# dfm/george

Measured on AMD Instinct MI355X. Metric: gp_compute_plus_log_likelihood_effective_tflops, higher is better.
Workload: dtype f64; 1 GPU; N=65536 1-D sorted uniform(0,10) x, var(y)*ExpSquaredKernel(1.0), yerr=0.1, dense Cholesky fp64 (BasicSolver path): compute()+log_likelihood(); N=65536, kernel=ExpSquared, solver=dense-cholesky, parallelism=1gpu

## Files before the change

### george_amd/_native.py

```python
import ctypes as C
import os

import numpy as np

_HERE = os.path.dirname(os.path.abspath(__file__))
LIB_PATH = os.path.join(_HERE, "csrc", "libgeorge_amd.so")

GH_MAX_AXES, GH_MAX_NDIM, GH_MAX_PARAMS, GH_MAX_METRIC = 8, 16, 4, 36
GH_MAX_NODES, GH_MAX_GRAD, GH_MAX_STACK = 64, 64, 8
GH_OK, GH_ERR_NOT_PD, GH_ERR_BAD_ARG, GH_ERR_HIP, GH_ERR_NOT_COMPUTED, GH_ERR_DIM, GH_ERR_NOMEM, GH_ERR_RANK = range(8)
GH_OP_LEAF, GH_OP_SUM, GH_OP_PRODUCT = 0, 1, 2


class gh_knode(C.Structure):
    _fields_ = [
        ("op", C.c_int32), ("kernel_type", C.c_int32), ("metric_type", C.c_int32),
        ("ndim", C.c_int32), ("naxes", C.c_int32), ("blocked", C.c_int32),
        ("n_params", C.c_int32), ("n_metric", C.c_int32),
        ("axes", C.c_int32 * GH_MAX_AXES),
        ("params", C.c_double * GH_MAX_PARAMS),
        ("constant", C.c_double),
        ("metric", C.c_double * GH_MAX_METRIC),
        ("min_block", C.c_double * GH_MAX_AXES),
        ("max_block", C.c_double * GH_MAX_AXES),
    ]


class gh_chol_opts(C.Structure):
    _fields_ = [("device", C.c_int32), ("nb", C.c_int32), ("profile", C.c_int32),
                ("lookahead", C.c_int32), ("reserved", C.c_int32 * 4)]


class gh_chol_profile(C.Structure):
    _fields_ = [("ms_total", C.c_double), ("ms_build", C.c_double), ("ms_panel", C.c_double),
                ("ms_trailing", C.c_double), ("trailing_flops", C.c_double), ("n_trailing", C.c_int64),
                ("ms_solve", C.c_double), ("ms_update_union", C.c_double), ("update_flops", C.c_double),
                ("reserved", C.c_double * 2)]


class gh_hodlr_opts(C.Structure):
    _fields_ = [("device", C.c_int32), ("min_size", C.c_int32), ("seed", C.c_int32),
                ("max_rank", C.c_int32), ("tol", C.c_double), ("reserved", C.c_int32 * 4)]


class gh_mgpu_opts(C.Structure):
    _fields_ = [("n_dev", C.c_int32), ("devices", C.c_int32 * 16), ("pr", C.c_int32), ("pc", C.c_int32),
                ("nb", C.c_int32), ("transport", C.c_int32), ("flags", C.c_int32), ("reserved", C.c_int32 * 3)]


class gh_hodlr_mgpu_opts(C.Structure):
    _fields_ = [("n_dev", C.c_int32), ("devices", C.c_int32 * 16), ("min_size", C.c_int32), ("seed", C.c_int32),
                ("max_rank", C.c_int32), ("tol", C.c_double), ("reserved", C.c_int32 * 4)]


GH_MGPU_RCCL, GH_MGPU_COPY = 0, 1
GH_MGPU_PLAIN_CYCLIC, GH_MGPU_CHAIN_ONLY, GH_MGPU_TRACE, GH_MGPU_ONE_COMM = 1, 2, 4, 8

if not os.path.exists(LIB_PATH):
    raise ImportError(
        "george_amd: %s not found -- build the HIP extension first "
        "(python -c 'import __graft_entry__ as g; g.build()' or make -C george_amd/csrc)" % LIB_PATH)

def _share_hip_runtime_with_torch():
    if os.environ.get("GEORGE_AMD_HIP_RUNTIME", "") == "system":
        return
    try:
        import importlib.util
        spec = importlib.util.find_spec("torch")
        if spec is None or not spec.submodule_search_locations:
            return
        cand = os.path.join(list(spec.submodule_search_locations)[0], "lib", "libamdhip64.so")
        if os.path.exists(cand):
            C.CDLL(cand, mode=C.RTLD_GLOBAL)
    except Exception:
        pass


_share_hip_runtime_with_torch()
lib = C.CDLL(LIB_PATH)

_vp, _dp, _i64, _i32 = C.c_void_p, C.c_void_p, C.c_int64, C.c_int32

SIGNATURES = {
    "gh_device_count": (C.c_int, []),
    "gh_last_error": (C.c_char_p, []),
    "gh_version": (C.c_char_p, []),
    "gh_release_caches": (None, [C.c_int32]),
    "gh_set_cache_limit": (None, [C.c_int64]),
    "gh_microbench_mfma_f64": (C.c_int, [C.POINTER(C.c_double)]),
    "gh_microbench_hbm_copy": (C.c_int, [C.POINTER(C.c_double)]),
    "gh_debug_set_mfma": (C.c_int, [C.c_int]),
    "gh_debug_set_gemm_sp": (C.c_int, [C.c_int]),
    "gh_debug_set_adaptive_panels": (C.c_int, [C.c_int]),
    "gh_debug_set_build_on_chain": (C.c_int, [C.c_int]),
    "gh_debug_set_gemm_grouped": (C.c_int, [C.c_int]),
    "gh_debug_set_hodlr_passes": (C.c_int, [C.c_int]),
    "gh_debug_set_hodlr_leaf_gj": (C.c_int, [C.c_int]),
    "gh_debug_set_hodlr_wave_aca": (C.c_int, [C.c_int]),
    "gh_debug_set_hodlr_coop_wgs": (C.c_int, [C.c_int]),
    "gh_debug_set_hodlr_coop_lower": (C.c_int, [C.c_int]),
    "gh_debug_set_hodlr_lpt": (C.c_int, [C.c_int]),
    "gh_debug_set_hodlr_u_from_v": (C.c_int, [C.c_int]),
    "gh_debug_set_hodlr_core_fused": (C.c_int, [C.c_int]),
    "gh_debug_set_hodlr_coop_singles": (C.c_int, [C.c_int]),
    "gh_debug_set_hodlr_leaf_fused": (C.c_int, [C.c_int]),
    "gh_debug_set_hodlr_strip_cols": (C.c_int, [C.c_int]),
    "gh_debug_stream_overlap": (C.c_int, [_vp, C.POINTER(C.c_double), C.c_int]),
    "gh_debug_stream_dispatch": (C.c_int, [_vp, C.POINTER(C.c_double), C.c_int]),
    "gh_microbench_suite": (C.c_int, [C.POINTER(C.c_double), C.c_int]),
    "gh_microbench_mfma_f64_ceiling": (C.c_int, [C.POINTER(C.c_double), C.c_int]),
    "gh_kernel_create": (C.c_int, [C.POINTER(gh_knode), C.c_int, C.POINTER(_vp)]),
    "gh_kernel_destroy": (None, [_vp]),
    "gh_kernel_ndim": (C.c_int, [_vp]),
    "gh_kernel_size": (C.c_int, [_vp]),
    "gh_kernel_value_general": (C.c_int, [_vp, _dp, _i64, _dp, _i64, _dp]),
    "gh_kernel_value_symmetric": (C.c_int, [_vp, _dp, _i64, _dp]),
    "gh_kernel_value_diagonal": (C.c_int, [_vp, _dp, _dp, _i64, _dp]),
    "gh_kernel_gradient_general": (C.c_int, [_vp, _dp, _dp, _i64, _dp, _i64, _dp]),
    "gh_kernel_gradient_symmetric": (C.c_int, [_vp, _dp, _dp, _i64, _dp]),
    "gh_kernel_x1_gradient_general": (C.c_int, [_vp, _dp, _i64, _dp, _i64, _dp]),
    "gh_kernel_x2_gradient_general": (C.c_int, [_vp, _dp, _i64, _dp, _i64, _dp]),
    "gh_chol_create": (C.c_int, [C.POINTER(gh_chol_opts), C.POINTER(_vp)]),
    "gh_chol_destroy": (None, [_vp]),
    "gh_chol_compute": (C.c_int, [_vp, _vp, _dp, _i64, _i32, _dp, C.POINTER(C.c_double)]),
    "gh_chol_info": (_i64, [_vp]),
    "gh_chol_size": (_i64, [_vp]),
    "gh_chol_device_bytes": (_i64, [_vp]),
    "gh_chol_solve": (C.c_int, [_vp, _dp, _i64, _dp]),
    "gh_chol_dot_solve": (C.c_int, [_vp, _dp, C.POINTER(C.c_double)]),
    "gh_chol_apply_sqrt": (C.c_int, [_vp, _dp, _i64, _dp]),
    "gh_chol_get_inverse": (C.c_int, [_vp, _dp]),
    "gh_chol_predict": (C.c_int, [_vp, _vp, _dp, _dp, _i64, _dp, _dp, _dp]),
    "gh_chol_grad": (C.c_int, [_vp, _vp, _dp, _dp, _dp, _dp, _dp]),
    "gh_chol_objective": (C.c_int, [_vp, _vp, _dp, _i64, _i32, _dp, _dp, _dp, C.POINTER(C.c_double), C.POINTER(C.c_double),
                                    _dp, _dp, _dp]),
    "gh_chol_objective_batch": (C.c_int, [_vp, _vp, _dp, _i32, _dp, _i64, _i32, _dp, _dp, _dp, _dp, _dp]),
    "gh_chol_predict_batch": (C.c_int, [_vp, _vp, _dp, _i32, _dp, _i64, _i32, _dp, _dp, _dp, _i64, _dp, _dp, _dp, _dp, _dp,
                                        _dp]),
    "gh_chol_objective_grad_batch": (C.c_int, [_vp, _vp, _dp, _i32, _dp, _i64, _i32, _dp, _dp, _dp, _dp, _dp, _dp, _dp,
                                               _dp, _dp]),
    "gh_chol_factor_size": (_i64, [_vp]),
    "gh_chol_dinv_size": (_i64, [_vp]),
    "gh_chol_export_factor": (C.c_int, [_vp, _dp, _dp]),
    "gh_chol_import_factor": (C.c_int, [_vp, _i64, _i32, _dp, _dp, _dp, C.c_double]),
    "gh_chol_trim": (None, [_vp]),
    "gh_chol_release_buffers": (None, [_vp]),
    "gh_chol_get_profile": (C.c_int, [_vp, C.POINTER(gh_chol_profile)]),
    "gh_chol_get_update_intervals": (C.c_int, [_vp, _dp, _i32, C.POINTER(C.c_int32)]),
    "gh_hodlr_create": (C.c_int, [C.POINTER(gh_hodlr_opts), C.POINTER(_vp)]),
    "gh_hodlr_destroy": (None, [_vp]),
    "gh_hodlr_compute": (C.c_int, [_vp, _vp, _dp, _i64, _i32, _dp, C.POINTER(C.c_double)]),
    "gh_hodlr_solve": (C.c_int, [_vp, _dp, _i64, _dp]),
    "gh_hodlr_dot_solve": (C.c_int, [_vp, _dp, C.POINTER(C.c_double)]),
    "gh_hodlr_get_inverse": (C.c_int, [_vp, _dp]),
    "gh_hodlr_ranks": (C.c_int, [_vp, C.POINTER(C.c_int32), _i32, C.POINTER(C.c_int32)]),
    "gh_hodlr_predict": (C.c_int, [_vp, _vp, _dp, _dp, _i64, _dp, _dp, _dp]),
    "gh_hodlr_grad": (C.c_int, [_vp, _vp, _dp, _dp, _dp, _dp, _dp]),
    "gh_mgpu_create": (C.c_int, [C.POINTER(gh_mgpu_opts), C.POINTER(_vp)]),
    "gh_mgpu_destroy": (None, [_vp]),
    "gh_mgpu_compute": (C.c_int, [_vp, _vp, _dp, _i64, _i32, _dp, C.POINTER(C.c_double)]),
    "gh_mgpu_info": (_i64, [_vp]),
    "gh_mgpu_grid": (C.c_int, [_vp, C.POINTER(C.c_int32), C.POINTER(C.c_int32), C.POINTER(C.c_int32)]),
    "gh_mgpu_comm_mode": (C.c_int, [_vp]),
    "gh_mgpu_dot_solve": (C.c_int, [_vp, _dp, C.POINTER(C.c_double)]),
    "gh_mgpu_solve": (C.c_int, [_vp, _dp, _i64, _dp]),
    "gh_mgpu_owner": (C.c_int, [_vp, _i64, _i64]),
    "gh_mgpu_apply_sqrt": (C.c_int, [_vp, _dp, _i64, _dp]),
    "gh_mgpu_get_inverse": (C.c_int, [_vp, _dp]),
    "gh_mgpu_predict": (C.c_int, [_vp, _vp, _dp, _dp, _i64, _dp, _dp, _dp]),
    "gh_mgpu_get_trace": (C.c_int, [_vp, _dp, _i64, C.POINTER(C.c_int64)]),
    "gh_hodlr_mgpu_create": (C.c_int, [C.POINTER(gh_hodlr_mgpu_opts), C.POINTER(_vp)]),
    "gh_hodlr_mgpu_destroy": (None, [_vp]),
    "gh_hodlr_mgpu_compute": (C.c_int, [_vp, _vp, _dp, _i64, _i32, _dp, C.POINTER(C.c_double)]),
    "gh_hodlr_mgpu_solve": (C.c_int, [_vp, _dp, _i64, _dp]),
    "gh_hodlr_mgpu_dot_solve": (C.c_int, [_vp, _dp, C.POINTER(C.c_double)]),
    "gh_hodlr_mgpu_ranks": (C.c_int, [_vp, C.POINTER(C.c_int32), _i32, C.POINTER(C.c_int32)]),
# ... 63 lines not shown
```

### george_amd/csrc/gh_chol.hip

```cpp
#include <math.h>
#include <string.h>
#include <algorithm>
#include <chrono>
#include "gh_common.h"
#include "gh_device_util.h"
#include "gh_spin.h"
#include "../../include/george_amd_debug.h"

#define T 128
#define LP 129

__global__ __launch_bounds__(256) void potf2_inv_kernel(double* A, long lda, double* dinv,
                                                        long long* info, long long base) {
  __shared__ double s[T * LP];
  __shared__ int fail_at;
  const int tid = threadIdx.x;
  if (*info != 0) return;
  if (tid == 0) fail_at = -1;
  for (int idx = tid; idx < T * T; idx += 256) {
    const int i = idx >> 7, j = idx & 127;
    s[i * LP + j] = A[(long)i * lda + j];
  }
  __syncthreads();
  const int ty = tid >> 4, tx = tid & 15;
  for (int j = 0; j < T; ++j) {
    const double d = s[j * LP + j];
    if (!(d > 0.0)) {
      if (tid == 0) fail_at = j;
      break;
    }
    const double ajj = sqrt(d);
    __syncthreads();
    if (tid < T) {
      if (tid > j) s[tid * LP + j] /= ajj;
      else if (tid == j) s[j * LP + j] = ajj;
    }
    __syncthreads();
    for (int i = j + 1 + ((ty - (j + 1)) & 15); i < T; i += 16) {
      const double lij = s[i * LP + j];
      for (int k = j + 1 + ((tx - (j + 1)) & 15); k <= i; k += 16)
        s[i * LP + k] -= lij * s[k * LP + j];
    }
    __syncthreads();
  }
  __syncthreads();
  if (fail_at >= 0) {
    if (tid == 0) *info = base + fail_at + 1;
    return;
  }
  for (int idx = tid; idx < T * T; idx += 256) {
    const int i = idx >> 7, j = idx & 127;
    A[(long)i * lda + j] = (j <= i) ? s[i * LP + j] : 0.0;
  }
  __syncthreads();
  {
    volatile double* vs = s;
    const int c = tid >> 1, h = tid & 1;
    const double xc = 1.0 / vs[c * LP + c];
    for (int i = c + 1; i < T; ++i) {
      double acc = (h == 0) ? vs[i * LP + c] * xc : 0.0;
      for (int k = c + 1 + h; k < i; k += 2) acc += vs[i * LP + k] * vs[c * LP + k];
      acc += __shfl_xor(acc, 1, 64);
      const double xi = -acc / vs[i * LP + i];
      if (h == 0) vs[c * LP + i] = xi;
    }
  }
  __syncthreads();
  for (int idx = tid; idx < T * T; idx += 256) {
    const int i = idx >> 7, j = idx & 127;
    double v;
    if (j < i) v = s[j * LP + i];
    else if (j == i) v = 1.0 / s[i * LP + i];
    else v = 0.0;
    dinv[idx] = v;
  }
}


__global__ __launch_bounds__(256) void logdet_kernel(const double* A, long lda, long n, double* out, int accumulate) {
  __shared__ double sh[4];
  double v = 0.0;
  for (long i = threadIdx.x; i < n; i += 256) v += log(A[i * lda + i]);
  v = block_sum_256(v, sh);
  if (threadIdx.x == 0) out[0] = (accumulate ? out[0] : 0.0) + 2.0 * v;
}
__global__ __launch_bounds__(256) void dot_kernel(const double* a, const double* b, long n, double* out, const int* fail) {
  __shared__ double sh[4];
  double v = 0.0;
  for (long i = threadIdx.x; i < n; i += 256) v += a[i] * b[i];
// ... 264 lines not shown
  }
  red[wave][2 * lane] = acc.x;
  red[wave][2 * lane + 1] = acc.y;
  __syncthreads();
  if (tid < T) {
    double v = 0.0;
#pragma unroll
    for (int q = 0; q < 8; ++q) v += red[q][tid];
    wv[tid] = zv - v;
  }
  __syncthreads();
  acc = make_double2(0.0, 0.0);
#pragma unroll
  for (int q = 0; q < 16; ++q) { const double wr = wv[wave * 16 + q]; acc.x += dv[q].x * wr; acc.y += dv[q].y * wr; }
  __syncthreads();
  red[wave][2 * lane] = acc.x;
  red[wave][2 * lane + 1] = acc.y;
  __syncthreads();
  if (tid < T) {
    double v = 0.0;
#pragma unroll
    for (int q = 0; q < 8; ++q) v += red[q][tid];
    if (!chain_ready(v)) v = __longlong_as_double(0x7FF8000000000000LL);
    __hip_atomic_store(x + (long)b * T + tid, v, __ATOMIC_RELAXED, __HIP_MEMORY_SCOPE_AGENT);
  }
}

__global__ __launch_bounds__(256) void colreduce_kernel(const double* V, long ldv, long nrows, long rows_per,
                                                        const double* z, double* pmu, double* pvar, long ncols_p) {
  const long c = (long)blockIdx.x * 256 + threadIdx.x;
  if (c >= ncols_p) return;
  const long r0 = (long)blockIdx.y * rows_per;
  const long r1 = r0 + rows_per < nrows ? r0 + rows_per : nrows;
  double am = 0.0, av = 0.0;
  for (long r = r0; r < r1; ++r) {
    const double v = V[r * ldv + c];
    am += v * z[r];
    av += v * v;
  }
  pmu[(long)blockIdx.y * ncols_p + c] = am;
  pvar[(long)blockIdx.y * ncols_p + c] = av;
}
__global__ void colfinal_kernel(const double* pmu, const double* pvar, long nchunks, long ncols_p, long m,
                                double* mu, double* var ) {
  const long c = (long)blockIdx.x * blockDim.x + threadIdx.x;
  if (c >= m) return;
  double am = 0.0, av = 0.0;
  for (long s = 0; s < nchunks; ++s) { am += pmu[s * ncols_p + c]; av += pvar[s * ncols_p + c]; }
  mu[c] = am;
  if (var) var[c] -= av;
}
__global__ void fill_kernel(double* p, long n, double v) {
  for (long i = (long)blockIdx.x * blockDim.x + threadIdx.x; i < n; i += (long)gridDim.x * blockDim.x) p[i] = v;
}
__global__ void eye_kernel(double* p, long n, long ld) {
  const long i = (long)blockIdx.x * blockDim.x + threadIdx.x;
  if (i < n) p[i * ld + i] = 1.0;
}
__global__ void symmetrize_kernel(const double* in, long ldi, double* out, long ldo, long n) {
  const long idx = (long)blockIdx.x * blockDim.x + threadIdx.x;
  if (idx >= n * n) return;
  const long i = idx / n, j = idx % n;
  out[i * ldo + j] = (j <= i) ? in[i * ldi + j] : in[j * ldi + i];
}
__global__ void copy2d_kernel(const double* in, long ldi, double* out, long ldo, long rows, long cols) {
  const long idx = (long)blockIdx.x * blockDim.x + threadIdx.x;
  if (idx >= rows * cols) return;
  const long i = idx / cols, j = idx % cols;
  out[i * ldo + j] = in[i * ldi + j];
}

struct EvPair { hipEvent_t a, b; };

struct gh_chol {
  gh_chol_opts opts;
  hipStream_t st = nullptr;
  hipStream_t st2 = nullptr;
  hipStream_t st3 = nullptr;
  bool shared_streams = false;
  hipStream_t st4 = nullptr;
  hipEvent_t ev_diag[32] = {};
  hipEvent_t ev_aux = nullptr, ev_aux2 = nullptr;
  std::vector<hipEvent_t> ev_p, ev_w, ev_nf;
  hipStream_t st_mask = nullptr;
  hipStream_t tail = nullptr;


  int mask_reserved = -1;
  hipEvent_t ev_xfer = nullptr;
  hipEvent_t ev_sync[3] = {nullptr, nullptr, nullptr};
  int64_t n = 0, np = 0;
  int ndim = 0;
  bool computed = false;
  int64_t info = 0;
  double logdet = 0.0;
  GhBuf A, dinv, x, yerr, v0, v1, v2, scal, rhs, work, work2, scratch, chain;
  long long* d_info = nullptr;
  bool build_on_chain = false;
  GhBatchBufs* batch = nullptr;
  gh_chol_profile prof;
  std::vector<EvPair> ev_pool;
  size_t ev_used = 0;
  std::vector<size_t> ev_trailing, ev_panel, ev_update;
  std::vector<double> ev_update_flops;
  std::vector<double> upd_intervals;
  long next_ev() {
    if (ev_used == ev_pool.size()) {
      EvPair p;
      if (hipEventCreate(&p.a) != hipSuccess || hipEventCreate(&p.b) != hipSuccess) return -1;
      ev_pool.push_back(p);
    }
    return (long)ev_used++;
  }
  ~gh_chol() {
    for (auto& p : ev_pool) { (void)hipEventDestroy(p.a); (void)hipEventDestroy(p.b); }
    for (auto& e : ev_sync) if (e) (void)hipEventDestroy(e);
    if (ev_xfer) (void)hipEventDestroy(ev_xfer);
    if (ev_aux) (void)hipEventDestroy(ev_aux);
    if (ev_aux2) (void)hipEventDestroy(ev_aux2);
    for (auto* v : {&ev_p, &ev_w, &ev_nf}) for (auto e : *v) (void)hipEventDestroy(e);
    for (auto& e : ev_diag) if (e) (void)hipEventDestroy(e);
    if (st4 && !shared_streams) (void)hipStreamDestroy(st4);
    if (st3 && !shared_streams) (void)hipStreamDestroy(st3);
    if (st_mask && !shared_streams) (void)hipStreamDestroy(st_mask);


    if (st2 && !shared_streams) (void)hipStreamDestroy(st2);
    if (st && !shared_streams) (void)hipStreamDestroy(st);
    gh_batch_free(batch);
  }
};

#include <map>
#include <mutex>
namespace {
struct SharedStreams {
  hipStream_t q[4] = {nullptr, nullptr, nullptr, nullptr};
  bool made = false;
  bool main_crowded = false;
  std::map<int, hipStream_t> masked;
};
std::mutex g_ss_mu;
std::map<int, SharedStreams> g_ss;
}
namespace {
__global__ void place_spin_kernel(long long ticks) {
  const long long t0 = wall_clock64();
  while (wall_clock64() - t0 < ticks) {}
}
double dispatch_wait_ms(hipStream_t big, hipStream_t small) {
  (void)hipDeviceSynchronize();
  hipLaunchKernelGGL(place_spin_kernel, dim3(1 << 17), dim3(64), 0, big, 5000LL);
  const auto t0 = std::chrono::steady_clock::now();
  hipLaunchKernelGGL(place_spin_kernel, dim3(1), dim3(64), 0, small, 0LL);
  (void)hipStreamSynchronize(small);
  const double ms = std::chrono::duration<double, std::milli>(std::chrono::steady_clock::now() - t0).count();
  (void)hipDeviceSynchronize();
  return ms;
}
}
bool gh_streams_dispatch_independently(hipStream_t a, hipStream_t b) {
  if (!a || !b || a == b) return false;
  hipLaunchKernelGGL(place_spin_kernel, dim3(1), dim3(64), 0, a, 0LL);
  hipLaunchKernelGGL(place_spin_kernel, dim3(1), dim3(64), 0, b, 0LL);
  (void)hipDeviceSynchronize();
  const bool ok = dispatch_wait_ms(a, b) <= 0.3 && dispatch_wait_ms(b, a) <= 0.3;
  (void)hipGetLastError();
  return ok;
}
bool gh_shared_main_crowded(int device) {
  std::lock_guard<std::mutex> lk(g_ss_mu);
  auto it = g_ss.find(device);
  return it != g_ss.end() && it->second.main_crowded;
}
bool gh_shared_streams(int device, hipStream_t q[4]) {
  std::lock_guard<std::mutex> lk(g_ss_mu);
  SharedStreams& ss = g_ss[device];
  if (!ss.made) {
    ss.made = true;
    if (hipSetDevice(device) != hipSuccess) { (void)hipGetLastError(); return false; }
    gh_prime_device(device);
    if (hipStreamCreate(&ss.q[0]) != hipSuccess) { ss.q[0] = nullptr; (void)hipGetLastError(); }
    int lo = 0, hi = 0;
    (void)hipDeviceGetStreamPriorityRange(&lo, &hi);
    for (int i = 1; i < 4 && ss.q[0]; ++i)
      if (hipStreamCreateWithPriority(&ss.q[i], hipStreamNonBlocking, hi) != hipSuccess) { ss.q[i] = nullptr; (void)hipGetLastError(); break; }
    if (ss.q[0] && ss.q[1] && ss.q[2] && ss.q[3]) {
      for (int i = 0; i < 4; ++i) hipLaunchKernelGGL(place_spin_kernel, dim3(1), dim3(64), 0, ss.q[i], 0LL);
      (void)hipDeviceSynchronize();
      for (int i = 1; i < 4 && !ss.main_crowded; ++i)
        ss.main_crowded = dispatch_wait_ms(ss.q[0], ss.q[i]) > 0.3 || dispatch_wait_ms(ss.q[i], ss.q[0]) > 0.3;
      (void)hipGetLastError();
    }
  }
  for (int i = 0; i < 4; ++i) q[i] = ss.q[i];
  return ss.q[0] != nullptr;
}
hipStream_t gh_shared_masked_stream(int device, int reserve_cus) {
  std::lock_guard<std::mutex> lk(g_ss_mu);
  SharedStreams& ss = g_ss[device];
  auto it = ss.masked.find(reserve_cus);
  if (it != ss.masked.end()) return it->second;
  hipStream_t st = nullptr;
// ... 170 lines not shown
      GH_CHECK(gemm_nt(st, P, ld, P, ld, dj, T, rem, T, T, 1.0, 0.0, false));
      GH_CHECK(gemm_nt(st, blk(A, ld, j0 + T, j0 + T), ld, P, ld, P, ld, rem, rem, T, -1.0, 1.0, true));
    }
  }
  return GH_OK;
}
static int trsm_right(hipStream_t st, const double* L11, int64_t ld11, const double* dinv, double* A21, int64_t lda, int64_t m, int64_t n) {
  for (int64_t j0 = 0; j0 < n; j0 += T) {
    double* Xj = A21 + j0;
    if (j0 > 0)
      GH_CHECK(gemm_nt(st, Xj, lda, A21, lda, L11 + j0 * ld11, ld11, m, T, j0, -1.0, 1.0, false));
    GH_CHECK(gemm_nt(st, Xj, lda, Xj, lda, dinv + (j0 / T) * T * T, T, m, T, T, 1.0, 0.0, false));
  }
  return GH_OK;
}

static int launch_trsv_fwd_chain(const double* L, long ld, const double* dinv, int64_t nt, const double* w, double* z,
                                 unsigned* flags, hipStream_t st) {
  GH_HIP(hipMemsetAsync(flags + nt, 0, sizeof(unsigned), st));
  GH_HIP(hipMemsetAsync(z, 0xFF, (size_t)nt * T * sizeof(double), st));
  hipLaunchKernelGGL(trsv_fwd_chain_direct, dim3((unsigned)nt), dim3(CHAIN_THREADS), 0, st, L, ld, dinv, w, z, (int*)(flags + nt));
  GH_HIP(hipGetLastError());
  return GH_OK;
}
static int launch_trsv_bwd_chain(const double* L, long ld, const double* dinv, int64_t nt, const double* w, double* x,
                                 unsigned* flags, hipStream_t st) {
  GH_HIP(hipMemsetAsync(flags + nt, 0, sizeof(unsigned), st));
  GH_HIP(hipMemsetAsync(x, 0xFF, (size_t)nt * T * sizeof(double), st));
  hipLaunchKernelGGL(trsv_bwd_chain_direct, dim3((unsigned)nt), dim3(CHAIN_THREADS), 0, st, L, ld, dinv, (int)nt, w, x, (int*)(flags + nt));
  GH_HIP(hipGetLastError());
  return GH_OK;
}
extern "C" int gh_dev_potrf_block(double* a, int64_t lda, int64_t n, double* dinv, int64_t* info_dev, int64_t base_index, void* stream) {
  if (n % T) { gh_set_error("potrf_block: n must be a multiple of 128"); return GH_ERR_BAD_ARG; }
  struct Guard { bool prev; Guard() : prev(t_gemm_small_lds) { t_gemm_small_lds = true; } ~Guard() { t_gemm_small_lds = prev; } } guard;
  return potrf_block((hipStream_t)stream, a, lda, n, dinv, (long long*)info_dev, base_index);
}
extern "C" int gh_dev_trsm_right(const double* l11, int64_t ld11, const double* dinv, double* a21, int64_t lda, int64_t m, int64_t n, void* stream) {
  if (n % T || m % T) { gh_set_error("trsm_right: sizes must be multiples of 128"); return GH_ERR_BAD_ARG; }
  struct Guard { bool prev; Guard() : prev(t_gemm_small_lds) { t_gemm_small_lds = true; } ~Guard() { t_gemm_small_lds = prev; } } guard;
  return trsm_right((hipStream_t)stream, l11, ld11, dinv, a21, lda, m, n);
}
extern "C" int gh_dev_trsv_lower(const double* l, int64_t ldl, const double* dinv, int64_t n,
                                 const double* w, double* z, void* scratch, void* stream) {
  if (n % T || n <= 0 || !scratch) { gh_set_error("trsv_lower: n must be a positive multiple of 128"); return GH_ERR_BAD_ARG; }
  const int64_t nt = n / T;
  if (w == z) { gh_set_error("trsv_lower: w and z must not be the same array"); return GH_ERR_BAD_ARG; }
  return launch_trsv_fwd_chain(l, (long)ldl, dinv, nt, w, z, (unsigned*)scratch, (hipStream_t)stream);
}
extern "C" int gh_dev_trsv_lower_t(const double* l, int64_t ldl, const double* dinv, int64_t n,
                                   const double* w, double* x, void* scratch, void* stream) {
  if (n % T || n <= 0 || !scratch) { gh_set_error("trsv_lower_t: n must be a positive multiple of 128"); return GH_ERR_BAD_ARG; }
  const int64_t nt = n / T;
  if (w == x) { gh_set_error("trsv_lower_t: w and x must not be the same array"); return GH_ERR_BAD_ARG; }
  return launch_trsv_bwd_chain(l, (long)ldl, dinv, nt, w, x, (unsigned*)scratch, (hipStream_t)stream);
}
extern "C" int gh_dev_logdet_accum(const double* a, int64_t lda, int64_t n, double* out_dev, void* stream) {
  hipLaunchKernelGGL(logdet_kernel, dim3(1), dim3(256), 0, (hipStream_t)stream, a, (long)lda, (long)n, out_dev, 1);
  GH_HIP(hipGetLastError());
  return GH_OK;
}

static int64_t panel_width(const gh_chol* s) {
  if (s->opts.nb > 0) return s->opts.nb;
  return 1024;
}
#ifndef GH_WIDE_PANEL_MIN_TRAILING
#define GH_WIDE_PANEL_MIN_TRAILING 25600
#endif

static int g_build_on_chain = 1;
extern "C" int gh_debug_set_build_on_chain(int on) {
  const int prev = g_build_on_chain;
  g_build_on_chain = on ? 1 : 0;
  return prev;
}
static int g_adaptive_panels = 1;
extern "C" int gh_debug_set_adaptive_panels(int on) {
  const int prev = g_adaptive_panels;
  g_adaptive_panels = on < 0 ? 1 : on;
  return prev;
}
static std::vector<int64_t> panel_starts(const gh_chol* s) {
  std::vector<int64_t> pc;
  const int64_t np = s->np, nb = panel_width(s);
  const bool adaptive = s->opts.nb == 0 && g_adaptive_panels && !use_simple_potf2();
  for (int64_t k0 = 0; k0 < np;) {
    pc.push_back(k0);
    const int64_t bound = g_adaptive_panels > 1 ? g_adaptive_panels : GH_WIDE_PANEL_MIN_TRAILING;
    int64_t w = (adaptive && np - (k0 + 2 * nb) >= bound) ? 2 * nb : nb;
#ifdef GH_WIDE_PANEL_TIER2
    if (adaptive && np - (k0 + 4 * nb) >= GH_WIDE_PANEL_TIER2) w = 4 * nb;
#endif
    k0 += std::min<int64_t>(w, np - k0);
  }
  pc.push_back(np);
  return pc;
}

static int panel_step(gh_chol* s, hipStream_t st, int64_t k0, int64_t nb) {
  double* A = s->A.d();
  const int64_t np = s->np, ld = np;
  double* dinv = s->dinv.d() + (k0 / T) * T * T;
  const int64_t m = np - (k0 + nb);
  const bool on_panel_stream = (st == s->st2);
  if (!s->st3 || !on_panel_stream || m <= 0 || nb / T > 32 || use_simple_potf2()) {
    GH_CHECK(potrf_block(st, blk(A, ld, k0, k0), ld, nb, dinv, s->d_info, k0));
    if (m > 0) {
      GH_CHECK(trsm_right(st, blk(A, ld, k0, k0), ld, dinv, blk(A, ld, k0 + nb, k0), ld, m, nb));
    }
    return GH_OK;
  }
  hipStream_t sa = s->st3;
  double* Ak = blk(A, ld, k0, k0);
  double* B = blk(A, ld, k0 + nb, k0);
  for (int64_t j0 = 0; j0 < nb; j0 += T) {
    double* dj = dinv + (j0 / T) * T * T;
    GH_CHECK(gh_launch_potf2_mfma(blk(Ak, ld, j0, j0), ld, dj, s->d_info, k0 + j0, st));
    GH_HIP(hipEventRecord(s->ev_diag[j0 / T], st));
    GH_HIP(hipStreamWaitEvent(sa, s->ev_diag[j0 / T], 0));
    double* Xj = B + j0;
    if (j0 > 0) GH_CHECK(gemm_nt(sa, Xj, ld, B, ld, Ak + j0 * ld, ld, m, T, j0, -1.0, 1.0, false));
    GH_CHECK(gemm_nt(sa, Xj, ld, Xj, ld, dj, T, m, T, T, 1.0, 0.0, false));
    const int64_t rem = nb - (j0 + T);
    if (rem > 0) {
      double* P = blk(Ak, ld, j0 + T, j0);
      GH_CHECK(gemm_nt(st, P, ld, P, ld, dj, T, rem, T, T, 1.0, 0.0, false));
      GH_CHECK(gemm_nt(st, blk(Ak, ld, j0 + T, j0 + T), ld, P, ld, P, ld, rem, rem, T, -1.0, 1.0, true));
    }
  }
  GH_HIP(hipEventRecord(s->ev_aux, sa));
  GH_HIP(hipStreamWaitEvent(st, s->ev_aux, 0));
  return GH_OK;
}

static hipStream_t trailing_stream(gh_chol* s) {
  int want = s->np < 24576 ? 32 : 0;
  if (const char* e = getenv("GEORGE_AMD_RESERVE_CUS")) want = atoi(e);
  if (want <= 0 || want >= 128) return s->st;
  if (s->mask_reserved != want) {
    if (s->st_mask) { (void)hipStreamSynchronize(s->st_mask); if (!s->shared_streams) (void)hipStreamDestroy(s->st_mask); s->st_mask = nullptr; }
    s->mask_reserved = want;
    hipDeviceProp_t prop;
    if (hipGetDeviceProperties(&prop, s->opts.device) == hipSuccess && prop.multiProcessorCount > 2 * want) {
      const int ncu = prop.multiProcessorCount, words = (ncu + 31) / 32;
      std::vector<uint32_t> mask(words, 0u);
      for (int c = want; c < ncu; ++c) mask[c / 32] |= (1u << (c % 32));
      if (s->shared_streams) s->st_mask = gh_shared_masked_stream(s->opts.device, want);
      else if (hipExtStreamCreateWithCUMask(&s->st_mask, words, mask.data()) != hipSuccess) { s->st_mask = nullptr; (void)hipGetLastError(); }
    }
    if (s->st_mask && !s->ev_xfer && hipEventCreateWithFlags(&s->ev_xfer, hipEventDisableTiming) != hipSuccess) {
      (void)hipGetLastError(); if (!s->shared_streams) (void)hipStreamDestroy(s->st_mask); s->st_mask = nullptr;
    }
  }
  return s->st_mask ? s->st_mask : s->st;
}

static int factor_lookahead_deep(gh_chol* s, int depth) {
  hipStream_t sm = trailing_stream(s), sn = (depth == 1 && s->st3) ? s->st3 : s->st4;
  hipStream_t sp = s->st2;
#ifndef GH_FULLCHIP_MS
#define GH_FULLCHIP_MS 2.5
#endif
  const std::vector<int64_t> pc = panel_starts(s);
  auto wide_stream = [&](int j) -> hipStream_t {
    if (sm == s->st) return sm;
    const int cwj = j + depth + 1;
    if (j < 0 || cwj > (int)pc.size() - 2) return sm;
    const double m2 = (double)(s->np - pc[cwj]);
    const double ms = (m2 / T) * (m2 / T + 1.0) / 2.0 * 2.0 * T * T * (double)(pc[j + 1] - pc[j]) / 60e12 * 1e3;
    return ms > GH_FULLCHIP_MS ? s->st : sm;
  };
  hipStream_t sw_prev = nullptr;
  double* A = s->A.d();
  const int64_t np = s->np, ld = np;
  const int P = (int)pc.size() - 1;
  const bool prof = s->opts.profile != 0;
  while ((int)s->ev_p.size() < P) {
    hipEvent_t e[3];
    for (auto& x : e) GH_HIP(hipEventCreateWithFlags(&x, hipEventDisableTiming));
// ... 3 lines not shown
  auto nbc = [&](int c) { return pc[c + 1] - pc[c]; };
  auto narrow = [&](hipStream_t st, int j, int c) -> int {
    const double* Pj = blk(A, ld, c0(c), c0(j));
    const long eu = prof ? s->next_ev() : -1;
    if (eu >= 0) { GH_HIP(hipEventRecord(s->ev_pool[eu].a, st)); s->ev_update.push_back((size_t)eu); }
    GH_CHECK(gemm_nt(st, blk(A, ld, c0(c), c0(c)), ld, Pj, ld, Pj, ld, np - c0(c), nbc(c), nbc(j), -1.0, 1.0, false));
    if (eu >= 0) GH_HIP(hipEventRecord(s->ev_pool[eu].b, st));
    const double tr = (double)(np - c0(c)) / T, tc = (double)nbc(c) / T;
    const double fl = (tr * tc - tc * (tc - 1.0) / 2.0) * 2.0 * T * T * (double)nbc(j);
    s->prof.update_flops += fl;
    if (eu >= 0) s->ev_update_flops.push_back(fl);
    return GH_OK;
  };
  if (!s->build_on_chain) {
    GH_HIP(hipEventRecord(s->ev_sync[0], s->st));
    GH_HIP(hipStreamWaitEvent(sp, s->ev_sync[0], 0));
    GH_HIP(hipStreamWaitEvent(sn, s->ev_sync[0], 0));
    if (sm != s->st) GH_HIP(hipStreamWaitEvent(sm, s->ev_sync[0], 0));
  }
  for (int j = 0; j < P; ++j) {
    {
      const long ep = prof ? s->next_ev() : -1;
      if (ep >= 0) { GH_HIP(hipEventRecord(s->ev_pool[ep].a, sp)); s->ev_panel.push_back((size_t)ep); }
      t_gemm_small_lds = wide_stream(j >= 1 ? j - 1 : 0) == s->st;
      GH_CHECK(panel_step(s, sp, c0(j), nbc(j)));
      if (ep >= 0) GH_HIP(hipEventRecord(s->ev_pool[ep].b, sp));
      GH_HIP(hipEventRecord(s->ev_p[j], sp));
    }
    if (j + 1 >= P) break;
    const hipEvent_t prev = (j >= 1) ? (depth >= 2 ? s->ev_nf[j - 1] : s->ev_w[j - 1]) : nullptr;
    if (prev) GH_HIP(hipStreamWaitEvent(sp, prev, 0));
    GH_CHECK(narrow(sp, j, j + 1));
    const int last_near = std::min(j + depth, P - 1);
    if (j + 2 <= last_near || (depth >= 2 && j + 2 <= P - 1)) GH_HIP(hipStreamWaitEvent(sn, s->ev_p[j], 0));
    for (int c = j + 2; c <= last_near; ++c) {
      if (c == j + depth && j >= 1) GH_HIP(hipStreamWaitEvent(sn, s->ev_w[j - 1], 0));
      GH_CHECK(narrow(sn, j, c));
      if (c == j + 2) GH_HIP(hipEventRecord(s->ev_nf[j], sn));
    }
    if (depth >= 2 && j + 2 > last_near) GH_HIP(hipEventRecord(s->ev_nf[j], sn));
    const int cw = j + depth + 1;
    hipStream_t sw = wide_stream(j);
    if (sw_prev && sw_prev != sw && j >= 1) GH_HIP(hipStreamWaitEvent(sw, s->ev_w[j - 1], 0));
    sw_prev = sw;
    GH_HIP(hipStreamWaitEvent(sw, s->ev_p[j], 0));
    if (cw <= P - 1) {
      const int64_t kw = c0(cw), m2 = np - kw;
      const long et = prof ? s->next_ev() : -1;
      if (et >= 0) {
        GH_HIP(hipEventRecord(s->ev_pool[et].a, sw)); s->ev_trailing.push_back((size_t)et); s->ev_update.push_back((size_t)et);
        s->ev_update_flops.push_back((double)(m2 / T) * (m2 / T + 1) / 2.0 * 2.0 * T * T * (double)nbc(j));
      }
      const double* P2 = blk(A, ld, kw, c0(j));
      GH_CHECK(gemm_nt(sw, blk(A, ld, kw, kw), ld, P2, ld, P2, ld, m2, m2, nbc(j), -1.0, 1.0, true));
      if (et >= 0) GH_HIP(hipEventRecord(s->ev_pool[et].b, sw));
      const double tiles = (double)(m2 / T) * (m2 / T + 1) / 2.0;
      s->prof.trailing_flops += tiles * 2.0 * T * T * (double)nbc(j);
      s->prof.update_flops += tiles * 2.0 * T * T * (double)nbc(j);
      s->prof.n_trailing += 1;
    }
    GH_HIP(hipEventRecord(s->ev_w[j], sw));
  }
  const bool join_on_chain = !s->shared_streams || gh_shared_main_crowded(s->opts.device);
  if (sm != s->st && join_on_chain) {
    GH_HIP(hipEventRecord(s->ev_sync[2], sn));
    GH_HIP(hipStreamWaitEvent(sp, s->ev_sync[2], 0));
    GH_HIP(hipEventRecord(s->ev_xfer, sm));
    GH_HIP(hipStreamWaitEvent(sp, s->ev_xfer, 0));
    if (P >= 2) GH_HIP(hipStreamWaitEvent(sp, s->ev_w[P - 2], 0));
    s->tail = sp;
    return GH_OK;
  }
  GH_HIP(hipEventRecord(s->ev_sync[1], sp));
  GH_HIP(hipStreamWaitEvent(s->st, s->ev_sync[1], 0));
  GH_HIP(hipEventRecord(s->ev_sync[2], sn));
  GH_HIP(hipStreamWaitEvent(s->st, s->ev_sync[2], 0));
  if (sm != s->st) {
    GH_HIP(hipEventRecord(s->ev_xfer, sm));
    GH_HIP(hipStreamWaitEvent(s->st, s->ev_xfer, 0));
  }
  return GH_OK;
}

#ifndef GH_LOOKAHEAD_DEPTH
#define GH_LOOKAHEAD_DEPTH 1
#endif
static int lookahead_depth(const gh_chol* s) {
  return GH_LOOKAHEAD_DEPTH;
}

static int factor(gh_chol* s) {
  struct Guard { bool prev; Guard(bool v) : prev(t_gemm_small_lds) { t_gemm_small_lds = v; } ~Guard() { t_gemm_small_lds = prev; } }
      guard(s->opts.lookahead && s->st2 && trailing_stream(s) == s->st);
  if (s->opts.lookahead && s->st2 && s->st3 && s->st4 && s->np > panel_width(s)) return factor_lookahead_deep(s, lookahead_depth(s));
  hipStream_t st = s->st;
  double* A = s->A.d();
  const int64_t np = s->np, ld = np;
  const bool prof = s->opts.profile != 0;
  const std::vector<int64_t> pc = panel_starts(s);
  for (size_t pj = 0; pj + 1 < pc.size(); ++pj) {
    const int64_t k0 = pc[pj], nb = pc[pj + 1] - pc[pj];
    const long ep = prof ? s->next_ev() : -1;
    if (ep >= 0) { GH_HIP(hipEventRecord(s->ev_pool[ep].a, st)); s->ev_panel.push_back((size_t)ep); }
    GH_CHECK(potrf_block(st, blk(A, ld, k0, k0), ld, nb, s->dinv.d() + (k0 / T) * T * T, s->d_info, k0));
    const int64_t m = np - (k0 + nb);
    if (m > 0)
      GH_CHECK(trsm_right(st, blk(A, ld, k0, k0), ld, s->dinv.d() + (k0 / T) * T * T, blk(A, ld, k0 + nb, k0), ld, m, nb));
    if (ep >= 0) GH_HIP(hipEventRecord(s->ev_pool[ep].b, st));
    if (m > 0) {
      const long et = prof ? s->next_ev() : -1;
      if (et >= 0) { GH_HIP(hipEventRecord(s->ev_pool[et].a, st)); s->ev_trailing.push_back((size_t)et); }
      const double* P = blk(A, ld, k0 + nb, k0);
      GH_CHECK(gemm_nt(st, blk(A, ld, k0 + nb, k0 + nb), ld, P, ld, P, ld, m, m, nb, -1.0, 1.0, true));
      if (et >= 0) GH_HIP(hipEventRecord(s->ev_pool[et].b, st));
      const double tiles = (double)(m / T) * (m / T + 1) / 2.0;
      s->prof.trailing_flops += tiles * 2.0 * T * T * (double)nb;
      s->prof.n_trailing += 1;
    }
  }
  return GH_OK;
}

__global__ void prep_inputs_kernel(const double* xs, long nx, const double* es, long ne, double* xd, double* ed, long long* info) {
  const long i = (long)blockIdx.x * blockDim.x + threadIdx.x, stride = (long)gridDim.x * blockDim.x;
  for (long e = i; e < nx; e += stride) xd[e] = xs[e];
  for (long e = i; e < ne; e += stride) ed[e] = es[e];
  if (i == 0) *info = 0;
}

struct ComputeCtx { long e_all = -1, e_build = -1; };
static int compute_enqueue(gh_chol* s, gh_kernel* k, const double* x, int64_t n, int32_t ndim, const double* yerr, ComputeCtx& c) {
  if (!s || !k || !x || !yerr || n <= 0) { gh_set_error("bad argument to compute"); return GH_ERR_BAD_ARG; }
  if (ndim != k->ndim) { gh_set_error("dimension mismatch"); return GH_ERR_DIM; }
  GH_CHECK(set_device(s));
  GH_CHECK(k->upload());
  s->computed = false;
  s->info = 0;
  const int64_t np = gh_round_up(n, T);
  s->n = n; s->np = np; s->ndim = ndim;
  GH_CHECK(s->A.ensure((size_t)np * np * sizeof(double)));
  GH_CHECK(s->dinv.ensure((size_t)(np / T) * T * T * sizeof(double)));
  GH_CHECK(s->x.ensure((size_t)n * ndim * sizeof(double)));
  GH_CHECK(s->yerr.ensure((size_t)n * sizeof(double)));
  GH_CHECK(s->scal.ensure(256 * sizeof(double)));
  s->build_on_chain = g_build_on_chain && s->opts.lookahead && s->st2 && s->st3 && s->st4 && np > panel_width(s);
  hipStream_t st = s->build_on_chain ? s->st2 : s->st;
  memset(&s->prof, 0, sizeof(s->prof));
  s->ev_used = 0; s->ev_trailing.clear(); s->ev_panel.clear(); s->ev_update.clear(); s->ev_update_flops.clear();
  const bool prof = s->opts.profile != 0;
  c.e_all = prof ? s->next_ev() : -1;
  c.e_build = prof ? s->next_ev() : -1;
  if (c.e_all >= 0) GH_HIP(hipEventRecord(s->ev_pool[c.e_all].a, st));
  s->d_info = (long long*)(s->scal.d() + 2);
  if (gh_is_device_ptr(x) && gh_is_device_ptr(yerr)) {
    const long tot = (long)n * ndim;
    hipLaunchKernelGGL(prep_inputs_kernel, dim3((unsigned)std::min<long>((tot + 255) / 256, 1024)), dim3(256), 0, st,
                       x, tot, yerr, (long)n, s->x.d(), s->yerr.d(), s->d_info);
    GH_HIP(hipGetLastError());
  } else {
    GH_CHECK(gh_to_device(s->x.d(), x, (size_t)n * ndim, st));
    GH_CHECK(gh_to_device(s->yerr.d(), yerr, (size_t)n, st));
    GH_HIP(hipMemsetAsync(s->d_info, 0, sizeof(long long), st));
  }
  if (c.e_build >= 0) GH_HIP(hipEventRecord(s->ev_pool[c.e_build].a, st));
  GH_CHECK(gh_launch_kmat(k, s->x.d(), n, s->x.d(), n, s->yerr.d(), s->A.d(), np, np, np, 0, 0, true, true, st));
  if (c.e_build >= 0) GH_HIP(hipEventRecord(s->ev_pool[c.e_build].b, st));
  s->tail = s->st;
  GH_CHECK(factor(s));
  GH_CHECK(launch_logdet(s->A.d(), np, np, s->scal.d(), s->scal.d() + 8, s->tail));
  if (c.e_all >= 0) GH_HIP(hipEventRecord(s->ev_pool[c.e_all].b, s->tail));
  return GH_OK;
}
static int compute_finish(gh_chol* s, const ComputeCtx& c, double ld_host, long long info_host, double* logdet_out) {
  if (s->opts.profile && c.e_all >= 0 && c.e_build >= 0) {
    float ms = 0;
    GH_HIP(hipEventElapsedTime(&ms, s->ev_pool[c.e_all].a, s->ev_pool[c.e_all].b)); s->prof.ms_total = ms;
    GH_HIP(hipEventElapsedTime(&ms, s->ev_pool[c.e_build].a, s->ev_pool[c.e_build].b)); s->prof.ms_build = ms;
// ... 440 lines not shown
```

### include/george_amd_debug.h

```cpp
#ifndef GEORGE_AMD_DEBUG_H_
#define GEORGE_AMD_DEBUG_H_

#include "george_amd.h"

#ifdef __cplusplus
extern "C" {
#endif

int gh_microbench_mfma_f64(double* tflops_out);
int gh_debug_set_mfma(int mode);
int gh_debug_set_gemm_sp(int mode);
int gh_debug_set_gemm_grouped(int mode);
int gh_debug_set_build_on_chain(int on);
int gh_debug_set_adaptive_panels(int on);
int gh_debug_set_hodlr_passes(int mask);
int gh_debug_set_hodlr_leaf_gj(int on);
int gh_debug_set_hodlr_wave_aca(int on);
int gh_debug_set_hodlr_coop_wgs(int n);
int gh_debug_set_hodlr_coop_lower(int div);
int gh_debug_set_hodlr_lpt(int on);
int gh_debug_set_hodlr_u_from_v(int on);
int gh_debug_set_hodlr_core_fused(int on);
int gh_debug_set_hodlr_coop_singles(int on);
int gh_debug_set_hodlr_leaf_fused(int on);
int gh_debug_set_hodlr_strip_cols(int cols);
int gh_debug_stream_overlap(gh_chol* s, double* out, int n);
int gh_debug_stream_dispatch(gh_chol* s, double* out, int n);
int gh_microbench_hbm_copy(double* gbps_out);
int gh_microbench_suite(double* out, int n);
int gh_microbench_mfma_f64_ceiling(double* out, int n);

enum {
  GH_MGPU_CHAIN_ONLY   = 2,
  GH_MGPU_TRACE        = 4
};
int  gh_mgpu_get_trace(const gh_mgpu* h, double* out, int64_t max_rows, int64_t* n_rows);

#ifdef __cplusplus
}
#endif
#endif
```

Baseline: 71.71 TFLOP/s.

## Add two-level grouped panel schedule for lookahead Cholesky factorization

Adds a planner that groups consecutive panels and factors each group on a chain stream with left-looking intra-group updates. Meanwhile the far trailing update for the whole group runs as one large GEMM on the main stream, tied together by events. Group sizes come from a cost model with hard-coded throughput and link-latency constants, aiming to batch trailing updates into fewer, larger GEMMs while keeping the panel chain hidden behind them. This replaces the depth-1 lookahead path by default, which risks a longer critical path if the model's estimates are off.

```diff
diff --git a/george_amd/_native.py b/george_amd/_native.py
--- a/george_amd/_native.py
+++ b/george_amd/_native.py
@@ -92,6 +92,10 @@
     "gh_debug_set_mfma": (C.c_int, [C.c_int]),
     "gh_debug_set_gemm_sp": (C.c_int, [C.c_int]),
     "gh_debug_set_adaptive_panels": (C.c_int, [C.c_int]),
+    "gh_debug_set_update_group": (C.c_int, [C.c_int]),
+    "gh_debug_set_update_hide": (C.c_double, [C.c_double]),
+    "gh_debug_chol_plan": (C.c_int, [C.c_int64, C.c_int64, C.c_int64, C.c_int32, C.c_double, C.POINTER(C.c_int64), C.c_int32, C.POINTER(C.c_int32),
+                                     C.POINTER(C.c_int64), C.c_int32, C.POINTER(C.c_int32), C.POINTER(C.c_int32)]),
     "gh_debug_set_build_on_chain": (C.c_int, [C.c_int]),
     "gh_debug_set_gemm_grouped": (C.c_int, [C.c_int]),
     "gh_debug_set_hodlr_passes": (C.c_int, [C.c_int]),
diff --git a/george_amd/csrc/gh_chol.hip b/george_amd/csrc/gh_chol.hip
--- a/george_amd/csrc/gh_chol.hip
+++ b/george_amd/csrc/gh_chol.hip
@@ -5,6 +5,7 @@
 #include "gh_common.h"
 #include "gh_device_util.h"
 #include "gh_spin.h"
+#include "gh_chol_plan.h"
 #include "../../include/george_amd_debug.h"
 
 #define T 128
@@ -435,6 +436,8 @@
   hipEvent_t ev_diag[32] = {};
   hipEvent_t ev_aux = nullptr, ev_aux2 = nullptr;
   std::vector<hipEvent_t> ev_p, ev_w, ev_nf;
+  GhCholPlan plan;
+  std::vector<hipEvent_t> ev_plan;
   hipStream_t st_mask = nullptr;
   hipStream_t tail = nullptr;
 
@@ -471,7 +474,7 @@
     if (ev_xfer) (void)hipEventDestroy(ev_xfer);
     if (ev_aux) (void)hipEventDestroy(ev_aux);
     if (ev_aux2) (void)hipEventDestroy(ev_aux2);
-    for (auto* v : {&ev_p, &ev_w, &ev_nf}) for (auto e : *v) (void)hipEventDestroy(e);
+    for (auto* v : {&ev_p, &ev_w, &ev_nf, &ev_plan}) for (auto e : *v) (void)hipEventDestroy(e);
     for (auto& e : ev_diag) if (e) (void)hipEventDestroy(e);
     if (st4 && !shared_streams) (void)hipStreamDestroy(st4);
     if (st3 && !shared_streams) (void)hipStreamDestroy(st3);
@@ -808,20 +811,13 @@
   return prev;
 }
 static std::vector<int64_t> panel_starts(const gh_chol* s) {
-  std::vector<int64_t> pc;
-  const int64_t np = s->np, nb = panel_width(s);
   const bool adaptive = s->opts.nb == 0 && g_adaptive_panels && !use_simple_potf2();
-  for (int64_t k0 = 0; k0 < np;) {
-    pc.push_back(k0);
-    const int64_t bound = g_adaptive_panels > 1 ? g_adaptive_panels : GH_WIDE_PANEL_MIN_TRAILING;
-    int64_t w = (adaptive && np - (k0 + 2 * nb) >= bound) ? 2 * nb : nb;
+  const int64_t bound = g_adaptive_panels > 1 ? g_adaptive_panels : GH_WIDE_PANEL_MIN_TRAILING;
 #ifdef GH_WIDE_PANEL_TIER2
-    if (adaptive && np - (k0 + 4 * nb) >= GH_WIDE_PANEL_TIER2) w = 4 * nb;
+  return gh_plan_panel_starts(s->np, panel_width(s), adaptive ? bound : 0, GH_WIDE_PANEL_TIER2);
+#else
+  return gh_plan_panel_starts(s->np, panel_width(s), adaptive ? bound : 0);
 #endif
-    k0 += std::min<int64_t>(w, np - k0);
-  }
-  pc.push_back(np);
-  return pc;
 }
 
 static int panel_step(gh_chol* s, hipStream_t st, int64_t k0, int64_t nb) {
@@ -991,6 +987,86 @@
   return GH_OK;
 }
 
+#ifndef GH_UPDATE_GROUP_DEFAULT
+#define GH_UPDATE_GROUP_DEFAULT 2
+#endif
+static int g_update_group = GH_UPDATE_GROUP_DEFAULT;
+extern "C" int gh_debug_set_update_group(int gmax) {
+  const int prev = g_update_group;
+  g_update_group = gmax < 1 ? GH_UPDATE_GROUP_DEFAULT : gmax;
+  return prev;
+}
+static double g_update_hide = GH_PLAN_HIDE;
+extern "C" double gh_debug_set_update_hide(double hide) {
+  const double prev = g_update_hide;
+  g_update_hide = hide > 0.0 ? hide : GH_PLAN_HIDE;
+  return prev;
+}
+extern "C" int gh_debug_chol_plan(int64_t np, int64_t nb, int64_t bound, int32_t gmax, double hide, int64_t* panel_starts_out, int32_t max_starts,
+                                  int32_t* n_starts, int64_t* ops_out, int32_t max_ops, int32_t* n_ops, int32_t* n_events) {
+  if (np <= 0 || nb <= 0 || np % T || nb % T || gmax < 1 || !n_starts || !n_ops || (max_starts > 0 && !panel_starts_out) || (max_ops > 0 && !ops_out)) {
+    gh_set_error("chol_plan: Np and nb must be positive multiples of 128, the group maximum at least 1");
+    return GH_ERR_BAD_ARG;
+  }
+  const GhCholPlan pl = gh_plan_build(np, gh_plan_panel_starts(np, nb, bound), gmax, hide);
+  *n_starts = (int32_t)pl.pc.size();
+  *n_ops = (int32_t)pl.ops.size();
+  if (n_events) *n_events = pl.n_events;
+  for (int32_t i = 0; i < *n_starts && i < max_starts; ++i) panel_starts_out[i] = pl.pc[i];
+  for (int32_t i = 0; i < *n_ops && i < max_ops; ++i) {
+    const GhPlanOp& o = pl.ops[i];
+    const int64_t row[GH_PLAN_COLS] = {o.kind, o.stream, o.r0, o.r1, o.c0, o.c1, o.k0, o.k1, o.wait0, o.wait1, o.record, o.lower};
+    memcpy(ops_out + (size_t)i * GH_PLAN_COLS, row, sizeof(row));
+  }
+  return GH_OK;
+}
+static int factor_two_level(gh_chol* s) {
+  hipStream_t sm = s->st, sp = s->st2;
+  const std::vector<int64_t> pc = panel_starts(s);
+  if (s->plan.np != s->np || s->plan.gmax != g_update_group || s->plan.hide != g_update_hide || s->plan.pc != pc)
+    s->plan = gh_plan_build(s->np, pc, g_update_group, g_update_hide);
+  const GhCholPlan& pl = s->plan;
+  while ((int)s->ev_plan.size() < pl.n_events) {
+    hipEvent_t e;
+    GH_HIP(hipEventCreateWithFlags(&e, hipEventDisableTiming));
+    s->ev_plan.push_back(e);
+  }
+  double* A = s->A.d();
+  const int64_t ld = s->np;
+  const bool prof = s->opts.profile != 0;
+  if (!s->build_on_chain) {
+    GH_HIP(hipEventRecord(s->ev_sync[0], s->st));
+    GH_HIP(hipStreamWaitEvent(sp, s->ev_sync[0], 0));
+    GH_HIP(hipStreamWaitEvent(s->st3, s->ev_sync[0], 0));
+  }
+  for (const GhPlanOp& o : pl.ops) {
+    hipStream_t st = o.stream == GH_PLAN_MAIN ? sm : sp;
+    if (o.wait0 >= 0) GH_HIP(hipStreamWaitEvent(st, s->ev_plan[o.wait0], 0));
+    if (o.wait1 >= 0) GH_HIP(hipStreamWaitEvent(st, s->ev_plan[o.wait1], 0));
+    if (o.kind == GH_PLAN_PANEL) {
+      const long ep = prof ? s->next_ev() : -1;
+      if (ep >= 0) { GH_HIP(hipEventRecord(s->ev_pool[ep].a, st)); s->ev_panel.push_back((size_t)ep); }
+      GH_CHECK(panel_step(s, st, o.c0, o.c1 - o.c0));
+      if (ep >= 0) GH_HIP(hipEventRecord(s->ev_pool[ep].b, st));
+    } else if (o.kind != GH_PLAN_JOIN) {
+      const int64_t m = o.r1 - o.r0, n = o.c1 - o.c0, k = o.k1 - o.k0;
+      const double fl = gh_plan_trap_tiles(m, n) * 2.0 * T * T * (double)k;
+      const long eu = prof ? s->next_ev() : -1;
+      if (eu >= 0) {
+        GH_HIP(hipEventRecord(s->ev_pool[eu].a, st));
+        s->ev_update.push_back((size_t)eu); s->ev_update_flops.push_back(fl);
+        if (o.kind == GH_PLAN_F) s->ev_trailing.push_back((size_t)eu);
+      }
+      GH_CHECK(gemm_nt(st, blk(A, ld, o.r0, o.c0), ld, blk(A, ld, o.r0, o.k0), ld, blk(A, ld, o.c0, o.k0), ld, m, n, k, -1.0, 1.0, o.lower != 0));
+      if (eu >= 0) GH_HIP(hipEventRecord(s->ev_pool[eu].b, st));
+      s->prof.update_flops += fl;
+      if (o.kind == GH_PLAN_F) { s->prof.trailing_flops += fl; s->prof.n_trailing += 1; }
+    }
+    if (o.record >= 0) GH_HIP(hipEventRecord(s->ev_plan[o.record], st));
+  }
+  return GH_OK;
+}
+
 #ifndef GH_LOOKAHEAD_DEPTH
 #define GH_LOOKAHEAD_DEPTH 1
 #endif
@@ -1001,7 +1077,10 @@
 static int factor(gh_chol* s) {
   struct Guard { bool prev; Guard(bool v) : prev(t_gemm_small_lds) { t_gemm_small_lds = v; } ~Guard() { t_gemm_small_lds = prev; } }
       guard(s->opts.lookahead && s->st2 && trailing_stream(s) == s->st);
-  if (s->opts.lookahead && s->st2 && s->st3 && s->st4 && s->np > panel_width(s)) return factor_lookahead_deep(s, lookahead_depth(s));
+  if (s->opts.lookahead && s->st2 && s->st3 && s->st4 && s->np > panel_width(s)) {
+    if (g_update_group > 1 && lookahead_depth(s) == 1 && !use_simple_potf2() && trailing_stream(s) == s->st) return factor_two_level(s);
+    return factor_lookahead_deep(s, lookahead_depth(s));
+  }
   hipStream_t st = s->st;
   double* A = s->A.d();
   const int64_t np = s->np, ld = np;
diff --git a/george_amd/csrc/gh_chol_plan.h b/george_amd/csrc/gh_chol_plan.h
--- /dev/null
+++ b/george_amd/csrc/gh_chol_plan.h
@@ -0,0 +1,143 @@
+#ifndef GH_CHOL_PLAN_H_
+#define GH_CHOL_PLAN_H_
+#include <stdint.h>
+#include <algorithm>
+#include <vector>
+
+enum { GH_PLAN_PANEL = 0, GH_PLAN_L = 1, GH_PLAN_T = 2, GH_PLAN_F = 3, GH_PLAN_JOIN = 4 };
+enum { GH_PLAN_MAIN = 0, GH_PLAN_CHAIN = 1 };
+#define GH_PLAN_COLS 12
+
+struct GhPlanOp {
+  int64_t kind, stream;
+  int64_t r0, r1, c0, c1;
+  int64_t k0, k1;
+  int64_t wait0, wait1;
+  int64_t record;
+  int64_t lower;
+};
+struct GhCholPlan {
+  int64_t np = 0;
+  int gmax = 0;
+  double hide = 0.0;
+  std::vector<int64_t> pc;
+  std::vector<int> gs;
+  std::vector<GhPlanOp> ops;
+  int n_events = 0;
+};
+
+static inline std::vector<int64_t> gh_plan_panel_starts(int64_t np, int64_t nb, int64_t bound, int64_t tier2 = 0) {
+  std::vector<int64_t> pc;
+  for (int64_t k0 = 0; k0 < np;) {
+    pc.push_back(k0);
+    int64_t w = (bound > 0 && np - (k0 + 2 * nb) >= bound) ? 2 * nb : nb;
+    if (tier2 > 0 && bound > 0 && np - (k0 + 4 * nb) >= tier2) w = 4 * nb;
+    k0 += std::min<int64_t>(w, np - k0);
+  }
+  pc.push_back(np);
+  return pc;
+}
+
+static inline double gh_plan_trap_tiles(int64_t m, int64_t n) {
+  const double tm = (double)(m / 128), tn = (double)(n / 128);
+  return tn * (tn + 1.0) / 2.0 + (tm - tn) * tn;
+}
+
+#ifndef GH_PLAN_FAR_TFLOPS
+#define GH_PLAN_FAR_TFLOPS 66.0
+#endif
+#ifndef GH_PLAN_CHAIN_TFLOPS
+#define GH_PLAN_CHAIN_TFLOPS 45.0
+#endif
+#ifndef GH_PLAN_LINK_MS
+#define GH_PLAN_LINK_MS 0.6
+#endif
+#ifndef GH_PLAN_HIDE
+#define GH_PLAN_HIDE 1.2
+#endif
+static inline std::vector<int> gh_plan_groups(int64_t np, const std::vector<int64_t>& pc, int gmax, double hide) {
+  const int P = (int)pc.size() - 1;
+  std::vector<int> gs;
+  if (gmax <= 1) {
+    for (int j = 0; j <= P; ++j) gs.push_back(j);
+    return gs;
+  }
+  const double tile_fl = 2.0 * 128.0 * 128.0;
+  gs.push_back(0);
+  int a = 0, b = 1, prev = 1;
+  while (b < P) {
+    int g = std::min(std::min(gmax, 2 * prev), P - b);
+    for (; g > 1; --g) {
+      const int e = b + g;
+      const int64_t kg = pc[b] - pc[a];
+      const double far_ms = gh_plan_trap_tiles(np - pc[e], np - pc[e]) * tile_fl * (double)kg / (GH_PLAN_FAR_TFLOPS * 1e9);
+      double chain_fl = 0.0, links = 0.0;
+      for (int j = b; j < e; ++j) {
+        links += (double)((pc[j + 1] - pc[j] + 127) / 128);
+        if (j > b) chain_fl += gh_plan_trap_tiles(np - pc[j], pc[j + 1] - pc[j]) * tile_fl * (double)(pc[j] - pc[b]);
+      }
+      const int64_t wnext = std::min<int64_t>(pc[e] - pc[b], np - pc[e]);
+      chain_fl += gh_plan_trap_tiles(np - pc[e], wnext) * tile_fl * (double)(pc[e] - pc[b]);
+      const double chain_ms = links * GH_PLAN_LINK_MS + chain_fl / (GH_PLAN_CHAIN_TFLOPS * 1e9);
+      if (chain_ms <= hide * far_ms) break;
+    }
+    gs.push_back(b);
+    a = b; b += g; prev = g;
+  }
+  gs.push_back(P);
+  return gs;
+}
+
+static inline GhCholPlan gh_plan_build(int64_t np, const std::vector<int64_t>& pc, int gmax, double hide = GH_PLAN_HIDE) {
+  GhCholPlan pl;
+  if (!(hide > 0.0)) hide = GH_PLAN_HIDE;
+  pl.np = np; pl.gmax = gmax; pl.hide = hide; pl.pc = pc;
+  pl.gs = gh_plan_groups(np, pc, gmax, hide);
+  const int G = (int)pl.gs.size() - 1;
+  int nev = 0;
+  int64_t ev_far_prev = -1;
+  auto update = [&](int kind, int stream, int64_t c0, int64_t c1, int64_t k0, int64_t k1) {
+    GhPlanOp o{};
+    o.kind = kind; o.stream = stream; o.r0 = c0; o.r1 = np; o.c0 = c0; o.c1 = c1; o.k0 = k0; o.k1 = k1;
+    o.wait0 = o.wait1 = o.record = -1;
+    o.lower = gh_plan_trap_tiles(np - c0, c1 - c0) > 128.0 ? 1 : 0;
+    return o;
+  };
+  for (int i = 0; i < G; ++i) {
+    const int a = pl.gs[i], b = pl.gs[i + 1];
+    int64_t ev_panel = -1;
+    for (int j = a; j < b; ++j) {
+      if (j > a) pl.ops.push_back(update(GH_PLAN_L, GH_PLAN_CHAIN, pc[j], pc[j + 1], pc[a], pc[j]));
+      GhPlanOp p{};
+      p.kind = GH_PLAN_PANEL; p.stream = GH_PLAN_CHAIN;
+      p.r0 = pc[j]; p.r1 = np; p.c0 = pc[j]; p.c1 = pc[j + 1]; p.k0 = pc[j]; p.k1 = pc[j + 1];
+      p.wait0 = p.wait1 = p.record = -1; p.lower = 1;
+      if (j == b - 1) p.record = ev_panel = nev++;
+      pl.ops.push_back(p);
+    }
+    if (i + 1 < G) {
+      GhPlanOp t = update(GH_PLAN_T, GH_PLAN_CHAIN, pc[b], pc[pl.gs[i + 2]], pc[a], pc[b]);
+      t.wait0 = ev_far_prev;
+      pl.ops.push_back(t);
+      if (i + 2 < G) {
+        const int64_t cf = pc[pl.gs[i + 2]];
+        GhPlanOp f = update(GH_PLAN_F, GH_PLAN_MAIN, cf, np, pc[a], pc[b]);
+        f.lower = 1;
+        f.wait0 = ev_panel;
+        f.record = ev_far_prev = nev++;
+        pl.ops.push_back(f);
+      } else {
+        ev_far_prev = -1;
+      }
+    } else {
+      GhPlanOp jn{};
+      jn.kind = GH_PLAN_JOIN; jn.stream = GH_PLAN_MAIN;
+      jn.r0 = jn.r1 = jn.c0 = jn.c1 = jn.k0 = jn.k1 = np;
+      jn.wait0 = ev_panel; jn.wait1 = -1; jn.record = -1; jn.lower = 0;
+      pl.ops.push_back(jn);
+    }
+  }
+  pl.n_events = nev;
+  return pl;
+}
+#endif
diff --git a/include/george_amd_debug.h b/include/george_amd_debug.h
--- a/include/george_amd_debug.h
+++ b/include/george_amd_debug.h
@@ -13,6 +13,10 @@
 int gh_debug_set_gemm_grouped(int mode);
 int gh_debug_set_build_on_chain(int on);
 int gh_debug_set_adaptive_panels(int on);
+int gh_debug_set_update_group(int gmax);
+double gh_debug_set_update_hide(double hide);
+int gh_debug_chol_plan(int64_t np, int64_t nb, int64_t bound, int32_t gmax, double hide, int64_t* panel_starts_out, int32_t max_starts,
+                       int32_t* n_starts, int64_t* ops_out, int32_t max_ops, int32_t* n_ops, int32_t* n_events);
 int gh_debug_set_hodlr_passes(int mask);
 int gh_debug_set_hodlr_leaf_gj(int on);
 int gh_debug_set_hodlr_wave_aca(int on);
```

Result: faster. 72.75 TFLOP/s (median of 6 runs) (+1.4%).
